# anands-repo/hello

Hardware: AMD Instinct MI355X
Metric: candidate sites/sec (whole node) (higher is better)
Workload: dtype f32

## Files before the change

### hello_amd/csrc/engine.hip

```cpp
#include <hip/hip_runtime.h>

#include <cstdarg>
#include <cstdio>
#include <cstring>
#include <new>
#include <stdexcept>
#include <string>
#include <vector>

#include "../../include/hello_mi355x.h"
#include "kernels.h"

namespace {

thread_local std::string g_last_error;

int fail(int code, const char* fmt, ...) {
    char buf[512];
    va_list ap;
    va_start(ap, fmt);
    vsnprintf(buf, sizeof(buf), fmt, ap);
    va_end(ap);
    g_last_error = buf;
    return code;
}

// ... 100 lines not shown
    DevBuf d_feat_in, d_feat_out;
    DevBuf d_support;
    DevBuf d_evidence;
    hipStream_t own_stream = nullptr;
    hipStream_t last_stream = nullptr;
    hipEvent_t ev_staged = nullptr;
    hipEvent_t ev_start = nullptr, ev_stop = nullptr;
    bool staged_pending = false;
    bool timed = false;
    bool profiling = false;
    std::vector<std::vector<hipEvent_t>> prof_events;
    int prof_count = 0;
    int prof_filter = 0;
    int debug_op = -1;
    DevBuf d_debug;
    size_t debug_floats = 0;
    int stamp_mode = 0;
    DevBuf d_stamps;
    int32_t stamp_layout[5] = {0, 0, 0, 0, 0};

    int32_t *roff0 = nullptr, *roff1 = nullptr, *aoff = nullptr, *site_of_allele = nullptr;
    int32_t *allele_of_read0 = nullptr, *allele_of_read1 = nullptr;
    int32_t *group_slot0 = nullptr, *group_slot1 = nullptr, *slot_off0 = nullptr, *slot_off1 = nullptr;
    hello::ReadConvPlan plan0{1, 0, 0}, plan1{1, 0, 0};
    bool wide_trunk[2] = {false, false};
    int64_t* pair_off = nullptr;
};

namespace {

long long rows_of(int domain, int32_t S, int32_t A, int64_t R0, int64_t R1) {
    switch (domain) {
        case HELLO_ROWS_READS0: return R0;
        case HELLO_ROWS_READS1: return R1;
        case HELLO_ROWS_ALLELES: return A;
        case HELLO_ROWS_SITES: return S;
    }
    return -1;
}

const char* op_name(int kind) {
    static const char* const names[] = {"?", "conv1d", "maxpool", "segsum", "mix", "head", "concat", "add", "readconv_fused",
                                        "layernorm", "compressor_fused", "xattn_front"};
    return kind >= 1 && kind <= HELLO_OP_XATTN_FRONT ? names[kind] : names[0];
}

int validate_op_buffers(const hello_model_desc* d, const hello_op& o, int i) {
    auto domain_of = [&](int id) { return id == HELLO_BUF_READS0 ? (int)HELLO_ROWS_READS0 : id == HELLO_BUF_READS1 ? (int)HELLO_ROWS_READS1
// ... 332 lines not shown
            delete e;
            return fail(HELLO_ERR_MODEL, "a weight block runs past the end of the blob");
        }
    }
    e->scratch.resize(desc->n_buffers);
    hipError_t err = hipMalloc((void**)&e->d_weights, nbytes);
    if (err == hipSuccess) err = hipMemcpy(e->d_weights, folded_weights, nbytes, hipMemcpyHostToDevice);
    if (err == hipSuccess) err = hipStreamCreateWithFlags(&e->own_stream, hipStreamNonBlocking);
    if (err == hipSuccess) err = hipEventCreateWithFlags(&e->ev_staged, hipEventDisableTiming);
    if (err == hipSuccess) err = hipEventCreate(&e->ev_start);
    if (err == hipSuccess) err = hipEventCreate(&e->ev_stop);
    if (err != hipSuccess) {
        hello_engine_destroy(e);
        return fail(HELLO_ERR_HIP, "engine setup failed: %s", hipGetErrorString(err));
    }
    const int n_ops = (int)e->ops.size();
    e->n_lanes = lanes.n_lanes;
    e->partial_of.assign(n_ops, -1);
    int n_partial = e->n_lanes > 1 ? 0 : 2;
    for (int i = 0; i < n_ops; ++i)
        if (e->ops[i].kind == HELLO_OP_READCONV_FUSED)
            e->partial_of[i] = e->n_lanes > 1 ? n_partial++ : (e->ops[i].seg == HELLO_SEG_READS1_TO_ALLELES ? 1 : 0);
    e->d_partial.resize(n_partial);
    if (e->n_lanes > 1) {
        auto lane_of = [&](int i) { return lane_of_op(e->ops[i]); };
        e->op_waits = std::move(lanes.op_waits);
        e->lane_tail = std::move(lanes.lane_tail);
        const std::vector<char>& read_elsewhere = lanes.read_elsewhere;
        e->op_done.assign(n_ops, nullptr);
        e->lane_streams.assign(e->n_lanes, nullptr);
        for (int l = 1; l < e->n_lanes && err == hipSuccess; ++l) err = hipStreamCreateWithFlags(&e->lane_streams[l], hipStreamNonBlocking);
        for (int i = 0; i < n_ops && err == hipSuccess; ++i)
            if (read_elsewhere[i] || (lane_of(i) > 0 && e->lane_tail[lane_of(i)] == i)) err = hipEventCreateWithFlags(&e->op_done[i], hipEventDisableTiming);
        if (err == hipSuccess) err = hipEventCreateWithFlags(&e->ev_lanes_go, hipEventDisableTiming);
        if (err != hipSuccess) {
            hello_engine_destroy(e);
            return fail(HELLO_ERR_HIP, "lane setup failed: %s", hipGetErrorString(err));
        }
    }
    *out = e;
    return HELLO_OK;
} catch (...) {
    return hello::exception_status("hello_engine_create");
}

void hello_engine_destroy(hello_engine* e) {
    if (!e) return;
    (void)hipSetDevice(e->device);
    (void)hipDeviceSynchronize();
    for (auto& b : e->scratch) b.release();
    e->d_csr.release();
    e->h_csr.release();
    e->d_logits.release();
    e->d_meta.release();
    e->d_post.release();
    e->d_out_small.release();
    e->h_io.release();
    e->d_rcl0.release();
    e->d_rcl1.release();
    for (auto& b : e->d_partial) b.release();
    for (hipStream_t st : e->lane_streams)
        if (st) (void)hipStreamDestroy(st);
    for (hipEvent_t ev : e->op_done)
        if (ev) (void)hipEventDestroy(ev);
    if (e->ev_lanes_go) (void)hipEventDestroy(e->ev_lanes_go);
    e->d_feat_in.release();
    e->d_feat_out.release();
    e->d_support.release();
    e->d_evidence.release();
    e->d_debug.release();
    e->d_stamps.release();
    if (e->d_weights) (void)hipFree(e->d_weights);
    if (e->own_stream) (void)hipStreamDestroy(e->own_stream);
    if (e->ev_staged) (void)hipEventDestroy(e->ev_staged);
    if (e->ev_start) (void)hipEventDestroy(e->ev_start);
    if (e->ev_stop) (void)hipEventDestroy(e->ev_stop);
    for (auto& ring : e->prof_events)
        for (auto ev : ring)
            if (ev) (void)hipEventDestroy(ev);
    delete e;
}

void* hello_engine_stream(hello_engine* e) { return e ? (void*)e->own_stream : nullptr; }
// ... 88 lines not shown
    if (capacity < n) return fail(HELLO_ERR_ARG, "capacity %lld < %lld words", (long long)capacity, (long long)n);
    HIP_TRY(hipSetDevice(e->device));
    HIP_TRY(hipStreamSynchronize(e->last_stream ? e->last_stream : e->own_stream));
    HIP_TRY(hipMemcpy(out, e->d_stamps.p, (size_t)n * sizeof(uint64_t), hipMemcpyDeviceToHost));
    return HELLO_OK;
} catch (...) {
    return hello::exception_status("hello_engine_debug_read_stamps");
}

int hello_engine_debug_read(hello_engine* e, float* out, int64_t capacity, int64_t* n_floats) try {
    if (!e || !n_floats) return fail(HELLO_ERR_ARG, "NULL argument");
    *n_floats = (int64_t)e->debug_floats;
    if (!out) return HELLO_OK;
    if (e->debug_floats == 0) return fail(HELLO_ERR_ARG, "no forward has run since hello_engine_debug_capture");
    if (capacity < (int64_t)e->debug_floats) return fail(HELLO_ERR_ARG, "capacity %lld < %zu floats", (long long)capacity, e->debug_floats);
    HIP_TRY(hipSetDevice(e->device));
    HIP_TRY(hipStreamSynchronize(e->last_stream ? e->last_stream : e->own_stream));
    HIP_TRY(hipMemcpy(out, e->d_debug.p, e->debug_floats * sizeof(float), hipMemcpyDeviceToHost));
    return HELLO_OK;
} catch (...) {
    return hello::exception_status("hello_engine_debug_read");
}

static int stage_batch_indices(hello_engine* e, const int32_t* rpa0, const int32_t* rpa1,
                               const int32_t* aps, int32_t S, int32_t A, int64_t R0, int64_t R1,
                               bool two_tech, hipStream_t stream) {
    const int win = hello::readconv_supports_window(e->desc.window) ? e->desc.window : 150;
    const int G = hello::readconv_reads_per_group(win);
    if ((e->wide_trunk[0] || e->wide_trunk[1]) && hello::readconv_wide_reads_per_group() != G)
        return fail(HELLO_ERR_ARG, "internal: the wide trunk's group size differs from the read convolver's");
    const hello::ReadConvPlan plan0 = e->wide_trunk[0] ? hello::readconv_wide_plan(R0) : hello::readconv_plan(R0, win);
    const hello::ReadConvPlan plan1 = !two_tech ? hello::ReadConvPlan{1, 0, 0}
                                      : e->wide_trunk[1] ? hello::readconv_wide_plan(R1) : hello::readconv_plan(R1, win);
    const int64_t n_groups0 = plan0.bulk_wgs + plan0.rest_wgs, n_groups1 = plan1.bulk_wgs + plan1.rest_wgs;
    e->plan0 = plan0;
    e->plan1 = plan1;
    size_t bytes = 0;
    auto add = [&](size_t count, size_t elem) { bytes += (count * elem + 15) & ~size_t(15); };
    add(A + 1, 4); add(A + 1, 4); add(S + 1, 4); add(A, 4);
    add(R0, 4); add(R1, 4);
    add(n_groups0 + 1, 4); add(n_groups1 + 1, 4);
    add(A + 1, 4); add(A + 1, 4);
    add(S + 1, 8);
    if (e->staged_pending) {
        HIP_TRY(hipEventSynchronize(e->ev_staged));
        e->staged_pending = false;
    }
    if (e->h_csr.ensure(bytes)) return fail(HELLO_ERR_HIP, "pinned allocation of %zu bytes failed", bytes);
    if (bytes > e->d_csr.cap) {
        HIP_TRY(hipStreamSynchronize(stream));
        if (e->d_csr.ensure(bytes)) return fail(HELLO_ERR_HIP, "device allocation of %zu bytes failed", bytes);
    }
    char* hc = (char*)e->h_csr.p;
    char* hbase = hc;
    int32_t* h_roff0 = carve<int32_t>(hc, A + 1);
    int32_t* h_roff1 = carve<int32_t>(hc, A + 1);
    int32_t* h_aoff = carve<int32_t>(hc, S + 1);
    int32_t* h_soa = carve<int32_t>(hc, A);
    int32_t* h_aor0 = carve<int32_t>(hc, R0);
    int32_t* h_aor1 = carve<int32_t>(hc, R1);
    int32_t* h_gs0 = carve<int32_t>(hc, n_groups0 + 1);
    int32_t* h_gs1 = carve<int32_t>(hc, n_groups1 + 1);
    int32_t* h_so0 = carve<int32_t>(hc, A + 1);
    int32_t* h_so1 = carve<int32_t>(hc, A + 1);
    int64_t* h_poff = carve<int64_t>(hc, S + 1);

    auto build_reads = [&](const int32_t* rpa, int64_t R, int32_t* roff, int32_t* aor, int32_t* gslot,
                           int32_t* soff, const hello::ReadConvPlan& plan, const char* which) -> int {
        int64_t acc = 0;
        for (int32_t a = 0; a < A; ++a) {
            if (rpa[a] <= 0)
                return fail(HELLO_ERR_SHAPE, "%s[%d] = %d: every allele needs >= 1 read (dummy zero read)",
                            which, a, rpa[a]);
            roff[a] = (int32_t)acc;
            for (int32_t r = 0; r < rpa[a]; ++r) {
                if (acc + r < R) aor[acc + r] = a;
            }
            acc += rpa[a];
            if (acc > R) return fail(HELLO_ERR_SHAPE, "sum(%s) exceeds n_reads = %lld", which, (long long)R);
        }
        roff[A] = (int32_t)acc;
        if (acc != R)
            return fail(HELLO_ERR_SHAPE, "sum(%s) = %lld != n_reads = %lld", which, (long long)acc, (long long)R);
        const int64_t n_wgs = plan.bulk_wgs + plan.rest_wgs;
        const int64_t bulk_reads = plan.rest_wgs ? plan.bulk_wgs * plan.groups_per_wg * G : R;
        for (int32_t a = 0; a <= A; ++a) soff[a] = 0;
        int64_t slot = 0;
        for (int64_t w = 0; w < n_wgs; ++w) {
            int64_t r_lo, r_hi;
            if (w < plan.bulk_wgs) {
                r_lo = w * plan.groups_per_wg * G;
                r_hi = r_lo + (int64_t)plan.groups_per_wg * G;
                if (r_hi > bulk_reads) r_hi = bulk_reads;
            } else {
                r_lo = bulk_reads + (w - plan.bulk_wgs) * G;
                r_hi = r_lo + G < R ? r_lo + G : R;
            }
            if (r_lo >= r_hi) return fail(HELLO_ERR_ARG, "internal: empty workgroup in the read-convolver plan");
            gslot[w] = (int32_t)slot;
            const int32_t first = aor[r_lo], last = aor[r_hi - 1];
            for (int32_t a = first; a <= last; ++a) soff[a + 1] += 1;
            slot += (last - first + 1);
        }
        gslot[n_wgs] = (int32_t)slot;
        int64_t s = 0;
        for (int32_t a = 0; a < A; ++a) {
            const int32_t count = soff[a + 1];
            soff[a] = (int32_t)s;
            s += count;
        }
        soff[A] = (int32_t)s;
        if (s != slot) return fail(HELLO_ERR_ARG, "internal: slot accounting mismatch");
        return 0;
    };
    if (int rc = build_reads(rpa0, R0, h_roff0, h_aor0, h_gs0, h_so0, plan0, "reads_per_allele0")) return rc;
    if (two_tech) {
        if (int rc = build_reads(rpa1, R1, h_roff1, h_aor1, h_gs1, h_so1, plan1, "reads_per_allele1")) return rc;
    } else {
        h_gs1[0] = 0;
    }
    int64_t acc = 0, pacc = 0;
    for (int32_t s = 0; s < S; ++s) {
        if (aps[s] <= 0) return fail(HELLO_ERR_SHAPE, "alleles_per_site[%d] = %d", s, aps[s]);
        h_aoff[s] = (int32_t)acc;
        h_poff[s] = pacc;
        for (int32_t k = 0; k < aps[s] && acc + k < A; ++k) h_soa[acc + k] = s;
        acc += aps[s];
        pacc += (int64_t)aps[s] * (aps[s] + 1) / 2;
        if (acc > A) return fail(HELLO_ERR_SHAPE, "sum(alleles_per_site) exceeds n_alleles = %d", A);
    }
    h_aoff[S] = (int32_t)acc;
    h_poff[S] = pacc;
    if (acc != A) return fail(HELLO_ERR_SHAPE, "sum(alleles_per_site) = %lld != n_alleles = %d", (long long)acc, A);

    HIP_TRY(hipMemcpyAsync(e->d_csr.p, hbase, bytes, hipMemcpyHostToDevice, stream));
    HIP_TRY(hipEventRecord(e->ev_staged, stream));
    e->staged_pending = true;
    char* dbase = (char*)e->d_csr.p;
    auto dev = [&](void* hp) { return dbase + ((char*)hp - hbase); };
    e->roff0 = (int32_t*)dev(h_roff0);
    e->roff1 = (int32_t*)dev(h_roff1);
    e->aoff = (int32_t*)dev(h_aoff);
    e->site_of_allele = (int32_t*)dev(h_soa);
    e->allele_of_read0 = (int32_t*)dev(h_aor0);
    e->allele_of_read1 = (int32_t*)dev(h_aor1);
    e->group_slot0 = (int32_t*)dev(h_gs0);
    e->group_slot1 = (int32_t*)dev(h_gs1);
    e->slot_off0 = (int32_t*)dev(h_so0);
    e->slot_off1 = (int32_t*)dev(h_so1);
    e->pair_off = (int64_t*)dev(h_poff);
    return 0;
}

int hello_engine_forward(hello_engine* e, const uint8_t* reads0, const int32_t* rpa0,
                         const uint8_t* reads1, const int32_t* rpa1, const int32_t* aps,
                         const uint8_t* ref_onehot, int32_t S, int32_t A, int64_t R0, int64_t R1,
                         float* logits, float* meta, float* posteriors, int32_t flags, void* hip_stream) try {
    if (!e) return fail(HELLO_ERR_ARG, "engine is NULL");
    const hello_model_desc& d = e->desc;
    const bool two_tech = d.channels1 > 0;
    if (S <= 0 || A <= 0 || R0 <= 0) return fail(HELLO_ERR_ARG, "empty batch (S=%d A=%d R0=%lld)", S, A, (long long)R0);
    if (A < S) return fail(HELLO_ERR_SHAPE, "n_alleles %d < n_sites %d", A, S);
    if (!reads0 || !rpa0 || !aps || !logits) return fail(HELLO_ERR_ARG, "NULL input/output pointer");
    if (two_tech && (!reads1 || !rpa1 || R1 <= 0)) return fail(HELLO_ERR_ARG, "model needs a second read set");
    if (!two_tech) R1 = 0;
    if (d.uses_ref && !ref_onehot) return fail(HELLO_ERR_ARG, "model needs ref_onehot");
    if (d.has_meta && !meta) return fail(HELLO_ERR_ARG, "model produces meta weights: meta output is NULL");
    if (R0 > 0x7fffffffLL || R1 > 0x7fffffffLL) return fail(HELLO_ERR_ARG, "more than 2^31 reads in one batch");
    HIP_TRY(hipSetDevice(e->device));
    hipStream_t stream = hip_stream ? (hipStream_t)hip_stream : e->own_stream;
// ... 241 lines not shown
                const bool t1 = o.seg == HELLO_SEG_READS1_TO_ALLELES;
                hello::ReadConvArgs a{};
                if (o.flags & HELLO_FLAG_SRC_U8) {
                    a.reads = (const uint8_t*)ptr(o.src0);
                    a.channels = o.cin;
                } else {
                    a.pooled = (const float*)ptr(o.src0);
                }
                if (!ptr(o.src0)) return fail(HELLO_ERR_ARG, "op %d reads an input the caller did not supply", op_index);
                a.w = e->d_weights + o.w_off;
                a.partial = (float*)e->d_partial[e->partial_of[op_index]].p;
                a.allele_of_read = t1 ? e->allele_of_read1 : e->allele_of_read0;
                a.slot_of_group = t1 ? e->group_slot1 : e->group_slot0;
                a.n_reads = t1 ? R1 : R0;
                a.window = d.window;
                a.softplus = (o.flags & HELLO_FLAG_SOFTPLUS) ? 1 : 0;
                a.extra_blocks = o.k;
                a.winograd = (o.flags & HELLO_FLAG_WINOGRAD) ? 1 : 0;
                a.bf16x3 = (o.flags & HELLO_FLAG_BF16X3) ? ((o.flags & HELLO_FLAG_BF16X3_32) ? 2 : 1) : 0;
                const bool wide = o.cout == 128;
                if ((size_t)o.w_off + (wide ? hello::readconv_wide_weight_floats() : hello::readconv_weight_floats(o.k, a.winograd, d.window)) +
                        (a.bf16x3 ? hello::readconv_bf16x3_extra_floats(o.k) : 0) > e->n_weight_floats)
                    return fail(HELLO_ERR_MODEL, "op %d: fused read-convolver weight block truncated", op_index);
                {
                    const hello::ReadConvPlan& plan = t1 ? e->plan1 : e->plan0;
                    const int G = hello::readconv_reads_per_group(d.window);
                    const long long total = a.n_reads;
                    const long long bulk_reads = plan.rest_wgs ? plan.bulk_wgs * plan.groups_per_wg * G : total;
                    a.groups_per_wg = plan.groups_per_wg;
                    a.n_reads = bulk_reads;
                    int32_t stamp_lay[5] = {0, 0, 0, 0, 0};
                    const int stamp_waves = hello::readconv_stamp_waves();
                    if ((e->stamp_mode & 1) && !t1 && total > 0) {
                        if (wide || !a.reads) return fail(HELLO_ERR_ARG, "stamps: the canonical fused read convolver from the bytes only");
                        const long long wgs = plan.rest_wgs ? plan.bulk_wgs + plan.rest_wgs : (long long)((total + (long long)G * plan.groups_per_wg - 1) / ((long long)G * plan.groups_per_wg));
                        const int slots = hello::readconv_stamp_slots();
                        const size_t bytes = (size_t)wgs * stamp_waves * plan.groups_per_wg * slots * sizeof(uint64_t);
                        if (bytes > e->d_stamps.cap) {
                            HIP_TRY(hipStreamSynchronize(stream));
                            if (e->d_stamps.ensure(bytes)) return fail(HELLO_ERR_HIP, "device allocation of %zu bytes failed", bytes);
                        }
                        HIP_TRY(hipMemsetAsync(e->d_stamps.p, 0, bytes, stream));
                        a.stamps = (unsigned long long*)e->d_stamps.p;
                        a.stamp_groups = plan.groups_per_wg;
                        a.stamp_mode = e->stamp_mode;
                        const int32_t lay[5] = {(int32_t)wgs, stamp_waves, plan.groups_per_wg, slots, (int32_t)(plan.rest_wgs ? plan.bulk_wgs : wgs)};
                        for (int i = 0; i < 5; ++i) stamp_lay[i] = lay[i];
                        e->stamp_layout[0] = 0;
                    }
                    HIP_TRY(wide ? hello::launch_readconv_wide(a, stream) : hello::launch_readconv_fused(a, stream));
                    if (plan.rest_wgs) {
                        hello::ReadConvArgs b = a;
                        if (b.stamps) b.stamps += (size_t)plan.bulk_wgs * stamp_waves * plan.groups_per_wg * hello::readconv_stamp_slots();
                        if (b.reads) b.reads += bulk_reads * d.window * o.cin;
                        else b.pooled += bulk_reads * (long long)o.lin * o.cin;
                        b.allele_of_read += bulk_reads;
                        b.slot_of_group += plan.bulk_wgs;
                        b.groups_per_wg = 1;
                        b.n_reads = total - bulk_reads;
                        HIP_TRY(wide ? hello::launch_readconv_wide(b, stream) : hello::launch_readconv_fused(b, stream));
                    }
                    if (a.stamps)
                        for (int i = 0; i < 5; ++i) e->stamp_layout[i] = stamp_lay[i];
                }
                HIP_TRY(hello::launch_readconv_finalize((const float*)e->d_partial[e->partial_of[op_index]].p, t1 ? e->slot_off1 : e->slot_off0,
                                                        (float*)ptr(o.dst), A, o.lout, o.cout, stream));
                break;
            }
        }
        if (op_index == e->debug_op) {
            const size_t per_row = o.kind == HELLO_OP_CONCAT ? (size_t)o.lout * (o.cin + o.c1)
                                   : (o.kind == HELLO_OP_CONV1D || o.kind == HELLO_OP_READCONV_FUSED || o.kind == HELLO_OP_COMPRESSOR_FUSED || o.kind == HELLO_OP_XATTN_FRONT) ? (size_t)o.lout * o.cout
                                   : (o.kind == HELLO_OP_MAXPOOL ? (size_t)o.lout * o.cin : (size_t)o.lin * o.cin);
            const size_t n = (size_t)rows * per_row;
            if (n * sizeof(float) > e->d_debug.cap) {
                HIP_TRY(hipStreamSynchronize(stream));
                if (e->d_debug.ensure(n * sizeof(float))) return fail(HELLO_ERR_HIP, "device allocation of %zu bytes failed", n * sizeof(float));
            }
            HIP_TRY(hipMemcpyAsync(e->d_debug.p, ptr(o.dst), n * sizeof(float), hipMemcpyDeviceToDevice, stream));
            e->debug_floats = n;
        }
        if (laned && e->op_done[op_index]) HIP_TRY(hipEventRecord(e->op_done[op_index], stream));
        ++op_index;
    }
// ... 318 lines not shown
```

### hello_amd/csrc/kernels.h

```cpp
#pragma once
#include <hip/hip_runtime.h>
#include <stdint.h>

namespace hello {

int device_cus();

struct ConvArgs {
    const void* src;
    const float* src2;
    int split;
    float* dst;
    const float* res;
    const float* w;
    const float* bias;
    long long m_total;
    int lin, lout, cin, cout, k, stride, pad;
    int cin_stride;
    int groups;
    int kpad;
    int cout_pad;
    int relu;
    int src_u8;
    unsigned wino_rows;
    int wino;
// ... 18 lines not shown

hipError_t launch_concat(const float* src0, const float* src1, float* dst, long long rows_x_len, int c0,
                         int c1, hipStream_t stream);

hipError_t launch_add(const float* src0, const float* src1, float* dst, long long n, hipStream_t stream);

hipError_t launch_layernorm(const float* src, const float* res, float* dst, const float* gamma, const float* beta,
                            long long positions, int c, float eps, int act, hipStream_t stream);

hipError_t launch_rcl_to_rlc(const uint8_t* src, uint8_t* dst, long long rows, int len, int c,
                             hipStream_t stream);

hipError_t launch_posteriors(const float* logits, const float* meta, const int32_t* allele_off,
                             const int64_t* pair_off, int n_sites, long long n_alleles, int n_experts,
                             long long n_pairs_total, float* out, hipStream_t stream);

struct ReadConvArgs {
    const uint8_t* reads;
    const float* pooled;
    int channels;
    const float* w;
    float* partial;
    const int32_t* allele_of_read;
    const int32_t* slot_of_group;
    int groups_per_wg;
    long long n_reads;
    int extra_blocks;
    int winograd;
    int window;
    int softplus;
    int bf16x3;
    unsigned long long* stamps;
    int stamp_groups;
    int stamp_mode;
};
int readconv_stamp_slots();
int readconv_stamp_waves();
bool readconv_supports_window(int window);
int readconv_reads_per_group(int window);
int readconv_frame_rows(int window);
int readconv_groups_per_workgroup(long long n_reads, int window);
struct ReadConvPlan {
    int groups_per_wg;
    long long bulk_wgs;
    long long rest_wgs;
};
ReadConvPlan readconv_plan(long long n_reads, int window);
ReadConvPlan readconv_wide_plan(long long n_reads);
int readconv_weight_floats(int extra_blocks, bool winograd, int window);
int readconv_bf16x3_extra_floats(int extra_blocks);
bool readconv_supports_extra_blocks(int extra_blocks);
hipError_t launch_readconv_fused(const ReadConvArgs& a, hipStream_t stream);
hipError_t launch_readconv_finalize(const float* partial, const int32_t* slot_off, float* frames, int n_alleles,
                                    int frame_rows, int channels, hipStream_t stream);
int readconv_wide_weight_floats();
int readconv_wide_reads_per_group();
hipError_t launch_readconv_wide(const ReadConvArgs& a, hipStream_t stream);

struct CompressorArgs {
    const float* frames;
    float* dst;
    const float* w;
    long long n_items;
    int blocks;
    int items_per_wg;
};
int small_launch_items_per_wg(long long n_items, int most);
int compressor_weight_floats(int blocks);
bool compressor_supports_blocks(int blocks);
hipError_t launch_compressor_fused(const CompressorArgs& a, hipStream_t stream);
// ... 67 lines not shown
```

### hello_amd/csrc/readconv_fused.hip

```cpp
#include <cstdlib>
#include <type_traits>

#include "kernels.h"

namespace hello {

typedef float f32x4 __attribute__((ext_vector_type(4)));

namespace rc {

constexpr int S1_STEPS = 6;
template <bool WINO, bool F33 = false>
struct Offs {
    static constexpr int KT = WINO ? 4 : 3;
    static constexpr int W3232 = 2 * KT * 2 * 256, W3264 = 4 * 3 * 2 * 256, W3264S = 4 * 1 * 2 * 256;
    static constexpr int W6464 = 4 * KT * 4 * 256;
    static constexpr int W6464D = F33 ? 4 * 5 * 4 * 256 : W6464;
    static constexpr int W3232D = F33 ? 2 * 5 * 2 * 256 : W3232;
    static constexpr int OFF_B = 0;
    static constexpr int OFF_C1 = OFF_B + 6 * (W3232D + 32);
    static constexpr int OFF_SC = OFF_C1 + W3264 + 64;
    static constexpr int OFF_C2 = OFF_SC + W3264S + 64;
    static constexpr int OFF_D = OFF_C2 + W6464D + 64;
    static constexpr int W_TRUNK = OFF_D + 6 * (W6464D + 64);
// ... 44 lines not shown
    static constexpr int NSREG = cmax((T2 * 4 + NW_ - 1) / NW_, 2 * ((RS2 * G_ / 2 + 15) / 16));
    static constexpr int LDS_BYTES = cmax(2 * BUF_FLOATS * 4 + 64 + U8_BYTES,
                                          BUF_FLOATS * 4 + (T2 * 16 + 2) * 256 + 64);
};
}

using Geometry = rc::Cfg<4, 4, 150>;
using Geometry250 = rc::Cfg<2, 4, 250>;
using GeometrySoftplus = rc::Cfg<4, 4, 150, rc::ACT_SOFTPLUS>;
static_assert(Geometry::F33 && GeometrySoftplus::F33 && !Geometry250::F33, "weight packing rule of readconv_pack.py");
static_assert(Geometry::F33_32 && GeometrySoftplus::F33_32, "weight packing rule of readconv_pack.py");
int readconv_bf16x3_extra_floats(int extra_blocks) { return (1 + 2 * (3 + extra_blocks)) * 12288 + 6 * 3072; }
int readconv_weight_floats(int extra_blocks, bool winograd, int window) {
    if (!winograd) return rc::Offs<false>::off_d(3 + extra_blocks);
    return window == 150 ? rc::Offs<true, true>::off_d(3 + extra_blocks) : rc::Offs<true>::off_d(3 + extra_blocks);
}
bool readconv_supports_extra_blocks(int extra_blocks) { return extra_blocks == 0 || extra_blocks == 2; }

bool readconv_supports_window(int window) { return window == 150 || window == 250; }
int readconv_reads_per_group(int window) { return window == 250 ? Geometry250::G : Geometry::G; }
int readconv_stamp_slots() { return rc::STAMP_SLOTS; }
int readconv_stamp_waves() { return Geometry::NW; }
int readconv_frame_rows(int window) { return window == 250 ? Geometry250::L2 : Geometry::L2; }
int readconv_groups_per_workgroup(long long n_reads, int window) {
    const long long slots = 2LL * device_cus();
    const int G = readconv_reads_per_group(window);
    const long long groups = (n_reads + G - 1) / G;
    int best = 1;
    double best_cost = 1e300;
    for (int n = 1; n <= 8; ++n) {
        const long long wgs = (groups + n - 1) / n;
        const double cost = (double)((wgs + slots - 1) / slots) * n * (n > 1 ? 0.988 : 1.0);
        if (cost <= best_cost) {
            best_cost = cost;
            best = n;
        }
    }
    return best;
}

ReadConvPlan readconv_plan(long long n_reads, int window) {
    const long long slots = 2LL * device_cus();
    const int G = readconv_reads_per_group(window);
    const long long groups = (n_reads + G - 1) / G;
    ReadConvPlan best{1, groups, 0};
    double best_cost = 1e300;
    for (int n = 1; n <= 8; ++n) {
        const long long rounds = (groups / n) / slots;
        if (rounds == 0) continue;
        const long long bulk = rounds * slots, rest = groups - bulk * n;
        const double cost = (double)rounds * n * (n > 1 ? 0.988 : 1.0) + (double)((rest + slots - 1) / slots);
        if (cost <= best_cost) {
            best_cost = cost;
            best = ReadConvPlan{n, bulk, rest};
        }
    }
    if (best_cost == 1e300) {
        const int n = readconv_groups_per_workgroup(n_reads, window);
        best = ReadConvPlan{n, (groups + n - 1) / n, 0};
    }
    return best;
}

template <int C>
__device__ __forceinline__ int swz(int row) {
    return (C == 64 || C == 128) ? 2 * (row & 7) : (C == 32 ? 2 * ((row >> 1) & 3) : 2 * ((row >> 2) & 1));
}

enum { SW_OLD = 0, SW_W = 1, SW_3 = 2, SW_SPLIT = 3, SW_GLOBAL = 4 };

typedef short bf16x8 __attribute__((ext_vector_type(8)));
typedef short bf16x4 __attribute__((ext_vector_type(4)));
__device__ __forceinline__ int split_off(int row, int g, int part) { return row * 256 + 16 * ((g + 8 * part) ^ (2 * (row & 7))); }
__device__ __forceinline__ unsigned short to_bf16(float x) {
    const __bf16 h = (__bf16)x;
    return __builtin_bit_cast(unsigned short, h);
}
__device__ __forceinline__ int split_off32(int row, int g, int part) { return row * 128 + 16 * ((g + 4 * part) ^ (2 * ((row >> 1) & 3))); }
__device__ __forceinline__ void split4(f32x4 v, bf16x4& h, bf16x4& l) {
#pragma unroll
    for (int e = 0; e < 4; ++e) {
        const unsigned short hi = to_bf16(v[e]);
        h[e] = (short)hi;
        l[e] = (short)to_bf16(v[e] - __uint_as_float((unsigned)hi << 16));
    }
// ... 1000 lines not shown
    {
        const int j = tid0 & 15;
        const int pg1 = wave0 / 2;
        if (WINO) {
#pragma unroll
            for (int k = 0; k < (T1 / 2 + 1) / 2; ++k) {
                pad1 |= ((((pg1 + 2 * k) * 16 + j) % (RS1 / 2)) == RS1 / 2 - 1 ? 1u : 0u) << k;
                pad1f |= ((((1 - pg1 + 2 * k) * 16 + j) % (RS1 / 2)) == RS1 / 2 - 1 ? 1u : 0u) << k;
            }
        } else {
#pragma unroll
            for (int k = 0; k < T1 / 2; ++k) pad1 |= ((((pg1 + 2 * k) * 16 + j) % RS1) >= L1 ? 1u : 0u) << k;
        }
    }

    float* const X = STEM ? bufB : bufA;
    float* const H = STEM ? bufA : bufB;
    f32x4 sreg[CF::NSREG];
    f32x4 wA[NVA], wB[NVB], w2[2];
    f32x4 w3[2][5];
    f32x4 (&w6)[6] = reinterpret_cast<f32x4 (&)[6]>(wA);
    f32x4 (&w12)[12] = reinterpret_cast<f32x4 (&)[12]>(wB);

    const long long wg_read0 = (long long)blockIdx.x * G * a.groups_per_wg;
    const int slot0 = a.slot_of_group[blockIdx.x];
    const int first_allele = a.allele_of_read[wg_read0];
    int cur = first_allele;
    constexpr int NF = (L2 * 16 + THREADS - 1) / THREADS;
    f32x4 carry[NF];
#pragma unroll
    for (int i = 0; i < NF; ++i) carry[i] = f32x4{0.f, 0.f, 0.f, 0.f};
    auto flush = [&]() {
#pragma unroll
        for (int i = 0; i < NF; ++i) {
            const int f = tid0 + THREADS * i;
            if (f < L2 * 16)
                *(f32x4*)(a.partial + ((long long)(slot0 + cur - first_allele) * L2 + (f >> 4)) * 64 + 4 * (f & 15)) = carry[i];
            carry[i] = f32x4{0.f, 0.f, 0.f, 0.f};
        }
    };

    for (int grp = 0; grp < a.groups_per_wg; ++grp) {
    int opaque_zero;
    asm volatile("s_mov_b32 %0, 0" : "=s"(opaque_zero));
    const int tid = tid0 + opaque_zero;
    const int wave = __builtin_amdgcn_readfirstlane(wave0 + opaque_zero);
    const int lane = tid & 63;
    const int cb2 = wave % 2, cb4 = wave;
    const long long read0 = wg_read0 + (long long)grp * G;
    if (read0 >= a.n_reads) break;
    unsigned long long* const stamp_base = STAMP ? a.stamps + (((long long)blockIdx.x * CF::NW + wave) * a.stamp_groups + grp) * STAMP_SLOTS : nullptr;
    auto stamp = [&](int slot) {
        if constexpr (STAMP) {
            const unsigned long long t = __builtin_amdgcn_s_memtime();
            if (grp < a.stamp_groups && lane == 0) stamp_base[slot] = t;
        }
    };
    auto barrier = [&](int id) {
        stamp(1 + 2 * id);
        __syncthreads();
        stamp(2 + 2 * id);
    };
    if constexpr (STAMP) {
        stamp(0);
        const unsigned long long rt = __builtin_amdgcn_s_memrealtime();
        const unsigned hw = __builtin_amdgcn_s_getreg((31 << 11) | 4), xcc = __builtin_amdgcn_s_getreg((31 << 11) | 20);
        if (grp < a.stamp_groups && lane == 0) {
            stamp_base[41] = (unsigned long long)hw | ((unsigned long long)xcc << 32);
            stamp_base[42] = rt;
        }
    }
    const int n_here = (int)((a.n_reads - read0) < G ? (a.n_reads - read0) : G);
    if constexpr (F33) {
        static_assert(!F33 || CF::F33_32, "the F(3,3) kernel runs its 32-channel blocks in F(3,3) form too");
// ... 211 lines not shown
            else
                wino_layer<CF, 64, MODE_RESID_INPLACE, false>(H, X, wB, nullptr, W + off_b + W6464, pad2w, dump, wave, lane);
        } else {
            conv_layer<CF, 64, 64, 3, 1, 1, RS2, RS2, L2, T2, MODE_PLAIN, true, GEOM_TRUNK, 16, RS2 * CF::G, true>(
                X, H, w12, slice(off_b, cb4, 12), W + off_a + W6464, sreg, pad2, dump, wave, lane);
            barrier(13 + 2 * blk);
            if (blk < NB64 - 1)
                conv_layer<CF, 64, 64, 3, 1, 1, RS2, RS2, L2, T2, MODE_RESID_INPLACE, true, GEOM_TRUNK, 16, RS2 * CF::G, true>(
                    H, X, w12, slice(O::off_d(blk + 1), cb4, 12), W + off_b + W6464, sreg, pad2, dump, wave, lane);
            else
                conv_layer<CF, 64, 64, 3, 1, 1, RS2, RS2, L2, T2, MODE_RESID_INPLACE, false, GEOM_TRUNK, 16, RS2 * CF::G, true>(
                    H, X, w12, nullptr, W + off_b + W6464, sreg, pad2, dump, wave, lane);
        }
        barrier(14 + 2 * blk);
    }

    static_assert(G <= 4, "the allele select below");
    int allele_of[G];
#pragma unroll
    for (int rd = 0; rd < G; ++rd) {
        const long long r = read0 + rd < a.n_reads ? read0 + rd : a.n_reads - 1;
        allele_of[rd] = __builtin_amdgcn_readfirstlane(a.allele_of_read[r]);
    }
#pragma nounroll
    for (int rd = 0; rd < n_here; ++rd) {
        const int al = rd == 0 ? allele_of[0] : rd == 1 ? allele_of[1 % G] : rd == 2 ? allele_of[2 % G] : allele_of[3 % G];
        if (al != cur) {
            flush();
            cur = al;
        }
#pragma unroll
        for (int i = 0; i < NF; ++i) {
            const int f = tid + THREADS * i;
            if (f < L2 * 16) {
                const f32x4 v = *(const f32x4*)(X + img_off<64, F33 ? SW_3 : SWX>(1 + rd * RS2 + (f >> 4), f & 15));
#pragma unroll
                for (int e = 0; e < 4; ++e) carry[i][e] += v[e];
            }
        }
    }
    barrier(19);
    if constexpr (STAMP) {
        const unsigned long long rt = __builtin_amdgcn_s_memrealtime();
        if (grp < a.stamp_groups && lane == 0) stamp_base[43] = rt;
    }
    }
    flush();
    if constexpr (STAMP) {
        static_assert(!STAMP || (NB64 == 3 && STEM && WINO && !BF16), "stamps: the default fp32 Winograd schedule (20 barriers per group)");
        const unsigned long long t = __builtin_amdgcn_s_memtime();
        if ((tid0 & 63) == 0) a.stamps[(((long long)blockIdx.x * CF::NW + wave0) * a.stamp_groups) * STAMP_SLOTS + 44] = t;
    }
}

template <class CF, int NB64, bool WINO, bool STEM_ONLY = false, bool BF16 = false, bool BF16_32 = false>
static hipError_t launch_cfg(const ReadConvArgs& a, hipStream_t stream) {
    static bool configured_on[64] = {};
    int dev = 0;
    if (hipGetDevice(&dev) != hipSuccess || dev < 0 || dev >= 64) return hipErrorInvalidDevice;
    bool& configured = configured_on[dev];
    if (!configured) {
        hipError_t e = hipSuccess;
        if constexpr (!STEM_ONLY)
            e = hipFuncSetAttribute((const void*)readconv_kernel<CF, false, NB64, WINO, BF16, BF16_32>,
                                    hipFuncAttributeMaxDynamicSharedMemorySize, CF::LDS_BYTES);
        if (e == hipSuccess)
            e = hipFuncSetAttribute((const void*)readconv_kernel<CF, true, NB64, WINO, BF16, BF16_32>,
                                    hipFuncAttributeMaxDynamicSharedMemorySize, CF::LDS_BYTES);
        if (e != hipSuccess) return e;
        configured = true;
    }
    if (a.groups_per_wg < 1) return hipErrorInvalidValue;
    const long long per_wg = (long long)CF::G * a.groups_per_wg;
    const unsigned groups = (unsigned)((a.n_reads + per_wg - 1) / per_wg);
    if (a.stamps) {
        if constexpr (std::is_same<CF, Geometry>::value && NB64 == 3 && WINO && !BF16 && !STEM_ONLY) {
            if (!a.reads || (a.channels != 6 && a.channels != 7) || a.stamp_groups < 1) return hipErrorInvalidValue;
            static bool stamped_on[64] = {};
            if (!stamped_on[dev]) {
                const hipError_t e = hipFuncSetAttribute((const void*)readconv_kernel<CF, true, NB64, WINO, false, false, true>,
                                                         hipFuncAttributeMaxDynamicSharedMemorySize, 100 * 1024);
                if (e != hipSuccess) return e;
                stamped_on[dev] = true;
            }
            const int lds = (a.stamp_mode & 2) ? 100 * 1024 : CF::LDS_BYTES;
            hipLaunchKernelGGL((readconv_kernel<CF, true, NB64, WINO, false, false, true>), dim3(groups), dim3(CF::THREADS), lds, stream, a);
            return hipGetLastError();
        } else {
            return hipErrorInvalidValue;
        }
    }
    if (a.reads) {
        if (a.channels != 6 && a.channels != 7) return hipErrorInvalidValue;
        hipLaunchKernelGGL((readconv_kernel<CF, true, NB64, WINO, BF16, BF16_32>), dim3(groups), dim3(CF::THREADS), CF::LDS_BYTES, stream, a);
    } else if constexpr (!STEM_ONLY) {
        hipLaunchKernelGGL((readconv_kernel<CF, false, NB64, WINO, BF16, BF16_32>), dim3(groups), dim3(CF::THREADS), CF::LDS_BYTES, stream, a);
    } else {
// ... 705 lines not shown
```

Before: 487,000.

## Replace static read-convolver workgroup plan with persistent chunked scheduling via atomic counter

The fused read convolver previously ran a bulk launch plus a remainder launch with a fixed number of groups per workgroup. It now builds a host-side list of chunks whose sizes taper toward the end, launches one persistent grid sized to the resident slots, and has each workgroup pull its next chunk from an atomic counter. This removes the second launch and aims to balance the tail across CUs. The cost is an extra memset and atomic per chunk, a loop around the kernel body that may raise register pressure, and an optional env cap on slots.

```diff
diff --git a/hello_amd/csrc/engine.hip b/hello_amd/csrc/engine.hip
--- a/hello_amd/csrc/engine.hip
+++ b/hello_amd/csrc/engine.hip
@@ -2,6 +2,7 @@
 
 #include <cstdarg>
 #include <cstdio>
+#include <cstdlib>
 #include <cstring>
 #include <new>
 #include <stdexcept>
@@ -148,8 +149,11 @@
     int32_t *roff0 = nullptr, *roff1 = nullptr, *aoff = nullptr, *site_of_allele = nullptr;
     int32_t *allele_of_read0 = nullptr, *allele_of_read1 = nullptr;
     int32_t *group_slot0 = nullptr, *group_slot1 = nullptr, *slot_off0 = nullptr, *slot_off1 = nullptr;
-    hello::ReadConvPlan plan0{1, 0, 0}, plan1{1, 0, 0};
     bool wide_trunk[2] = {false, false};
+    hello::ReadConvChunkPlan chunk_plan[2];
+    hello::ReadConvChunk* chunks[2] = {nullptr, nullptr};
+    int readconv_slots_cap = 0;
+    DevBuf d_counters;
     int64_t* pair_off = nullptr;
 };
 
@@ -528,6 +532,19 @@
         if (e->ops[i].kind == HELLO_OP_READCONV_FUSED)
             e->partial_of[i] = e->n_lanes > 1 ? n_partial++ : (e->ops[i].seg == HELLO_SEG_READS1_TO_ALLELES ? 1 : 0);
     e->d_partial.resize(n_partial);
+    if (e->d_counters.ensure((size_t)(n_ops > 0 ? n_ops : 1) * 64)) {
+        hello_engine_destroy(e);
+        return fail(HELLO_ERR_HIP, "device allocation of the chunk counters failed");
+    }
+    if (const char* cap = getenv("HELLO_READCONV_SLOTS")) {
+        char* end = nullptr;
+        const long v = strtol(cap, &end, 10);
+        if (end == cap || *end || v < 1 || v > (1 << 20)) {
+            hello_engine_destroy(e);
+            return fail(HELLO_ERR_ARG, "HELLO_READCONV_SLOTS = '%s': a count of resident workgroups >= 1", cap);
+        }
+        e->readconv_slots_cap = (int)v;
+    }
     if (e->n_lanes > 1) {
         auto lane_of = [&](int i) { return lane_of_op(e->ops[i]); };
         e->op_waits = std::move(lanes.op_waits);
@@ -565,6 +582,7 @@
     e->d_rcl0.release();
     e->d_rcl1.release();
     for (auto& b : e->d_partial) b.release();
+    e->d_counters.release();
     for (hipStream_t st : e->lane_streams)
         if (st) (void)hipStreamDestroy(st);
     for (hipEvent_t ev : e->op_done)
@@ -699,6 +717,11 @@
     return hello::exception_status("hello_engine_debug_read");
 }
 
+static long long readconv_slots(const hello_engine* e, int per_cu) {
+    const long long device = hello::readconv_resident_slots(per_cu);
+    return e->readconv_slots_cap > 0 && e->readconv_slots_cap < device ? e->readconv_slots_cap : device;
+}
+
 static int stage_batch_indices(hello_engine* e, const int32_t* rpa0, const int32_t* rpa1,
                                const int32_t* aps, int32_t S, int32_t A, int64_t R0, int64_t R1,
                                bool two_tech, hipStream_t stream) {
@@ -706,17 +729,19 @@
     const int G = hello::readconv_reads_per_group(win);
     if ((e->wide_trunk[0] || e->wide_trunk[1]) && hello::readconv_wide_reads_per_group() != G)
         return fail(HELLO_ERR_ARG, "internal: the wide trunk's group size differs from the read convolver's");
-    const hello::ReadConvPlan plan0 = e->wide_trunk[0] ? hello::readconv_wide_plan(R0) : hello::readconv_plan(R0, win);
-    const hello::ReadConvPlan plan1 = !two_tech ? hello::ReadConvPlan{1, 0, 0}
-                                      : e->wide_trunk[1] ? hello::readconv_wide_plan(R1) : hello::readconv_plan(R1, win);
-    const int64_t n_groups0 = plan0.bulk_wgs + plan0.rest_wgs, n_groups1 = plan1.bulk_wgs + plan1.rest_wgs;
-    e->plan0 = plan0;
-    e->plan1 = plan1;
+    const long long slots = readconv_slots(e, 2);
+    const int64_t groups0 = (R0 + G - 1) / G, groups1 = two_tech ? (R1 + G - 1) / G : 0;
+    const bool chunked0 = !e->wide_trunk[0], chunked1 = two_tech && !e->wide_trunk[1];
+    e->chunk_plan[0] = chunked0 ? hello::readconv_chunk_plan(groups0, slots) : hello::ReadConvChunkPlan{};
+    e->chunk_plan[1] = chunked1 ? hello::readconv_chunk_plan(groups1, slots) : hello::ReadConvChunkPlan{};
+    const int64_t n_groups0 = chunked0 ? 0 : groups0, n_groups1 = chunked1 ? 0 : groups1;
+    const int64_t n_chunks0 = e->chunk_plan[0].chunks, n_chunks1 = e->chunk_plan[1].chunks;
     size_t bytes = 0;
     auto add = [&](size_t count, size_t elem) { bytes += (count * elem + 15) & ~size_t(15); };
     add(A + 1, 4); add(A + 1, 4); add(S + 1, 4); add(A, 4);
     add(R0, 4); add(R1, 4);
     add(n_groups0 + 1, 4); add(n_groups1 + 1, 4);
+    add(n_chunks0, sizeof(hello::ReadConvChunk)); add(n_chunks1, sizeof(hello::ReadConvChunk));
     add(A + 1, 4); add(A + 1, 4);
     add(S + 1, 8);
     if (e->staged_pending) {
@@ -738,12 +763,14 @@
     int32_t* h_aor1 = carve<int32_t>(hc, R1);
     int32_t* h_gs0 = carve<int32_t>(hc, n_groups0 + 1);
     int32_t* h_gs1 = carve<int32_t>(hc, n_groups1 + 1);
+    hello::ReadConvChunk* h_ch0 = carve<hello::ReadConvChunk>(hc, n_chunks0);
+    hello::ReadConvChunk* h_ch1 = carve<hello::ReadConvChunk>(hc, n_chunks1);
     int32_t* h_so0 = carve<int32_t>(hc, A + 1);
     int32_t* h_so1 = carve<int32_t>(hc, A + 1);
     int64_t* h_poff = carve<int64_t>(hc, S + 1);
 
-    auto build_reads = [&](const int32_t* rpa, int64_t R, int32_t* roff, int32_t* aor, int32_t* gslot,
-                           int32_t* soff, const hello::ReadConvPlan& plan, const char* which) -> int {
+    auto build_reads = [&](const int32_t* rpa, int64_t R, int32_t* roff, int32_t* aor, int32_t* gslot, hello::ReadConvChunk* chunks,
+                           int64_t n_expected, int32_t* soff, const char* which) -> int {
         int64_t acc = 0;
         for (int32_t a = 0; a < A; ++a) {
             if (rpa[a] <= 0)
@@ -759,27 +786,31 @@
         roff[A] = (int32_t)acc;
         if (acc != R)
             return fail(HELLO_ERR_SHAPE, "sum(%s) = %lld != n_reads = %lld", which, (long long)acc, (long long)R);
-        const int64_t n_wgs = plan.bulk_wgs + plan.rest_wgs;
-        const int64_t bulk_reads = plan.rest_wgs ? plan.bulk_wgs * plan.groups_per_wg * G : R;
         for (int32_t a = 0; a <= A; ++a) soff[a] = 0;
-        int64_t slot = 0;
-        for (int64_t w = 0; w < n_wgs; ++w) {
-            int64_t r_lo, r_hi;
-            if (w < plan.bulk_wgs) {
-                r_lo = w * plan.groups_per_wg * G;
-                r_hi = r_lo + (int64_t)plan.groups_per_wg * G;
-                if (r_hi > bulk_reads) r_hi = bulk_reads;
-            } else {
-                r_lo = bulk_reads + (w - plan.bulk_wgs) * G;
-                r_hi = r_lo + G < R ? r_lo + G : R;
+        int64_t slot = 0, n_units = 0;
+        bool empty = false;
+        auto unit = [&](long long first_group, int n_groups) {
+            const int64_t r_lo = first_group * G, r_hi = r_lo + (int64_t)n_groups * G < R ? r_lo + (int64_t)n_groups * G : R;
+            if (r_lo >= r_hi) {
+                empty = true;
+                return;
             }
-            if (r_lo >= r_hi) return fail(HELLO_ERR_ARG, "internal: empty workgroup in the read-convolver plan");
-            gslot[w] = (int32_t)slot;
+            if (chunks) chunks[n_units] = hello::ReadConvChunk{(int32_t)first_group, (int32_t)n_groups, (int32_t)slot};
+            else gslot[n_units] = (int32_t)slot;
             const int32_t first = aor[r_lo], last = aor[r_hi - 1];
             for (int32_t a = first; a <= last; ++a) soff[a + 1] += 1;
             slot += (last - first + 1);
-        }
-        gslot[n_wgs] = (int32_t)slot;
+            n_units += 1;
+        };
+        const int64_t groups = (R + G - 1) / G;
+        if (chunks) {
+            hello::readconv_for_each_chunk(groups, slots, unit);
+            if (n_units != n_expected) return fail(HELLO_ERR_ARG, "internal: the read convolver's chunk list changed length");
+        } else {
+            for (int64_t w = 0; w < groups; ++w) unit(w, 1);
+            gslot[n_units] = (int32_t)slot;
+        }
+        if (empty) return fail(HELLO_ERR_ARG, "internal: empty chunk in the read-convolver plan");
         int64_t s = 0;
         for (int32_t a = 0; a < A; ++a) {
             const int32_t count = soff[a + 1];
@@ -790,9 +821,9 @@
         if (s != slot) return fail(HELLO_ERR_ARG, "internal: slot accounting mismatch");
         return 0;
     };
-    if (int rc = build_reads(rpa0, R0, h_roff0, h_aor0, h_gs0, h_so0, plan0, "reads_per_allele0")) return rc;
+    if (int rc = build_reads(rpa0, R0, h_roff0, h_aor0, h_gs0, chunked0 ? h_ch0 : nullptr, n_chunks0, h_so0, "reads_per_allele0")) return rc;
     if (two_tech) {
-        if (int rc = build_reads(rpa1, R1, h_roff1, h_aor1, h_gs1, h_so1, plan1, "reads_per_allele1")) return rc;
+        if (int rc = build_reads(rpa1, R1, h_roff1, h_aor1, h_gs1, chunked1 ? h_ch1 : nullptr, n_chunks1, h_so1, "reads_per_allele1")) return rc;
     } else {
         h_gs1[0] = 0;
     }
@@ -823,6 +854,8 @@
     e->allele_of_read1 = (int32_t*)dev(h_aor1);
     e->group_slot0 = (int32_t*)dev(h_gs0);
     e->group_slot1 = (int32_t*)dev(h_gs1);
+    e->chunks[0] = (hello::ReadConvChunk*)dev(h_ch0);
+    e->chunks[1] = (hello::ReadConvChunk*)dev(h_ch1);
     e->slot_off0 = (int32_t*)dev(h_so0);
     e->slot_off1 = (int32_t*)dev(h_so1);
     e->pair_off = (int64_t*)dev(h_poff);
@@ -1110,44 +1143,35 @@
                 if ((size_t)o.w_off + (wide ? hello::readconv_wide_weight_floats() : hello::readconv_weight_floats(o.k, a.winograd, d.window)) +
                         (a.bf16x3 ? hello::readconv_bf16x3_extra_floats(o.k) : 0) > e->n_weight_floats)
                     return fail(HELLO_ERR_MODEL, "op %d: fused read-convolver weight block truncated", op_index);
-                {
-                    const hello::ReadConvPlan& plan = t1 ? e->plan1 : e->plan0;
-                    const int G = hello::readconv_reads_per_group(d.window);
-                    const long long total = a.n_reads;
-                    const long long bulk_reads = plan.rest_wgs ? plan.bulk_wgs * plan.groups_per_wg * G : total;
-                    a.groups_per_wg = plan.groups_per_wg;
-                    a.n_reads = bulk_reads;
+                if (wide) {
+                    if ((e->stamp_mode & 1) && !t1) return fail(HELLO_ERR_ARG, "stamps: the canonical fused read convolver from the bytes only");
+                    a.groups_per_wg = 1;
+                    HIP_TRY(hello::launch_readconv_wide(a, stream));
+                } else {
+                    const hello::ReadConvChunkPlan& plan = e->chunk_plan[t1 ? 1 : 0];
+                    a.chunks = e->chunks[t1 ? 1 : 0];
+                    a.n_chunks = (int)plan.chunks;
+                    a.counter = (unsigned*)((char*)e->d_counters.p + (size_t)op_index * 64);
+                    const bool stamped = (e->stamp_mode & 1) && !t1 && a.n_reads > 0;
+                    a.resident_slots = (int)readconv_slots(e, stamped && (e->stamp_mode & 2) ? 1 : 2);
                     int32_t stamp_lay[5] = {0, 0, 0, 0, 0};
-                    const int stamp_waves = hello::readconv_stamp_waves();
-                    if ((e->stamp_mode & 1) && !t1 && total > 0) {
-                        if (wide || !a.reads) return fail(HELLO_ERR_ARG, "stamps: the canonical fused read convolver from the bytes only");
-                        const long long wgs = plan.rest_wgs ? plan.bulk_wgs + plan.rest_wgs : (long long)((total + (long long)G * plan.groups_per_wg - 1) / ((long long)G * plan.groups_per_wg));
-                        const int slots = hello::readconv_stamp_slots();
-                        const size_t bytes = (size_t)wgs * stamp_waves * plan.groups_per_wg * slots * sizeof(uint64_t);
+                    if (stamped) {
+                        if (!a.reads) return fail(HELLO_ERR_ARG, "stamps: the canonical fused read convolver from the bytes only");
+                        const int stamp_waves = hello::readconv_stamp_waves(), slots = hello::readconv_stamp_slots();
+                        const size_t bytes = (size_t)plan.chunks * stamp_waves * plan.head * slots * sizeof(uint64_t);
                         if (bytes > e->d_stamps.cap) {
                             HIP_TRY(hipStreamSynchronize(stream));
                             if (e->d_stamps.ensure(bytes)) return fail(HELLO_ERR_HIP, "device allocation of %zu bytes failed", bytes);
                         }
                         HIP_TRY(hipMemsetAsync(e->d_stamps.p, 0, bytes, stream));
                         a.stamps = (unsigned long long*)e->d_stamps.p;
-                        a.stamp_groups = plan.groups_per_wg;
+                        a.stamp_groups = plan.head;
                         a.stamp_mode = e->stamp_mode;
-                        const int32_t lay[5] = {(int32_t)wgs, stamp_waves, plan.groups_per_wg, slots, (int32_t)(plan.rest_wgs ? plan.bulk_wgs : wgs)};
+                        const int32_t lay[5] = {(int32_t)plan.chunks, stamp_waves, plan.head, slots, (int32_t)plan.bulk};
                         for (int i = 0; i < 5; ++i) stamp_lay[i] = lay[i];
                         e->stamp_layout[0] = 0;
                     }
-                    HIP_TRY(wide ? hello::launch_readconv_wide(a, stream) : hello::launch_readconv_fused(a, stream));
-                    if (plan.rest_wgs) {
-                        hello::ReadConvArgs b = a;
-                        if (b.stamps) b.stamps += (size_t)plan.bulk_wgs * stamp_waves * plan.groups_per_wg * hello::readconv_stamp_slots();
-                        if (b.reads) b.reads += bulk_reads * d.window * o.cin;
-                        else b.pooled += bulk_reads * (long long)o.lin * o.cin;
-                        b.allele_of_read += bulk_reads;
-                        b.slot_of_group += plan.bulk_wgs;
-                        b.groups_per_wg = 1;
-                        b.n_reads = total - bulk_reads;
-                        HIP_TRY(wide ? hello::launch_readconv_wide(b, stream) : hello::launch_readconv_fused(b, stream));
-                    }
+                    HIP_TRY(hello::launch_readconv_fused(a, stream));
                     if (a.stamps)
                         for (int i = 0; i < 5; ++i) e->stamp_layout[i] = stamp_lay[i];
                 }
diff --git a/hello_amd/csrc/kernels.h b/hello_amd/csrc/kernels.h
--- a/hello_amd/csrc/kernels.h
+++ b/hello_amd/csrc/kernels.h
@@ -1,6 +1,8 @@
 #pragma once
 #include <hip/hip_runtime.h>
 #include <stdint.h>
+
+#include "readconv_chunks.h"
 
 namespace hello {
 
@@ -65,6 +67,10 @@
     const float* w;
     float* partial;
     const int32_t* allele_of_read;
+    const ReadConvChunk* chunks;
+    int n_chunks;
+    unsigned* counter;
+    int resident_slots;
     const int32_t* slot_of_group;
     int groups_per_wg;
     long long n_reads;
@@ -82,13 +88,12 @@
 bool readconv_supports_window(int window);
 int readconv_reads_per_group(int window);
 int readconv_frame_rows(int window);
-int readconv_groups_per_workgroup(long long n_reads, int window);
 struct ReadConvPlan {
     int groups_per_wg;
     long long bulk_wgs;
     long long rest_wgs;
 };
-ReadConvPlan readconv_plan(long long n_reads, int window);
+long long readconv_resident_slots(int per_cu = 2);
 ReadConvPlan readconv_wide_plan(long long n_reads);
 int readconv_weight_floats(int extra_blocks, bool winograd, int window);
 int readconv_bf16x3_extra_floats(int extra_blocks);
diff --git a/hello_amd/csrc/readconv_chunks.h b/hello_amd/csrc/readconv_chunks.h
--- /dev/null
+++ b/hello_amd/csrc/readconv_chunks.h
@@ -0,0 +1,66 @@
+#pragma once
+
+#include <cstdint>
+
+namespace hello {
+
+constexpr int READCONV_MAX_CHUNK = 8;
+constexpr int READCONV_TAPER_ROUNDS = 2;
+
+struct ReadConvChunk {
+    int32_t first_group;
+    int32_t groups;
+    int32_t first_slot;
+};
+
+struct ReadConvChunkPlan {
+    int head = 1;
+    long long chunks = 0;
+    long long bulk = 0;
+    bool counter = false;
+};
+
+inline int readconv_head_groups(long long groups, long long slots) {
+    int best = 1;
+    double best_cost = 1e300;
+    for (int n = 1; n <= READCONV_MAX_CHUNK; ++n) {
+        const long long rounds = (groups / n) / slots;
+        if (rounds == 0) continue;
+        const long long rest = groups - rounds * slots * n;
+        const double cost = (double)rounds * n * (n > 1 ? 0.988 : 1.0) + (double)((rest + slots - 1) / slots);
+        if (cost <= best_cost) {
+            best_cost = cost;
+            best = n;
+        }
+    }
+    return best;
+}
+
+template <class F>
+inline ReadConvChunkPlan readconv_for_each_chunk(long long groups, long long slots, F&& f) {
+    ReadConvChunkPlan p;
+    if (groups <= 0) return p;
+    if (slots < 1) slots = 1;
+    p.head = readconv_head_groups(groups, slots);
+    const long long div = (long long)READCONV_TAPER_ROUNDS * slots;
+    int largest = 0;
+    for (long long g = 0; g < groups;) {
+        const long long left = groups - g;
+        long long n = (left + div - 1) / div;
+        if (n > p.head) n = p.head;
+        f(g, (int)n);
+        if ((int)n > largest) largest = (int)n;
+        p.chunks += 1;
+        p.bulk += n > 1;
+        g += n;
+    }
+    p.head = largest;
+    p.counter = p.chunks > slots;
+    return p;
+}
+
+inline ReadConvChunkPlan readconv_chunk_plan(long long groups, long long slots) {
+    return readconv_for_each_chunk(groups, slots, [](long long, int) {});
+}
+
+}
diff --git a/hello_amd/csrc/readconv_fused.hip b/hello_amd/csrc/readconv_fused.hip
--- a/hello_amd/csrc/readconv_fused.hip
+++ b/hello_amd/csrc/readconv_fused.hip
@@ -90,45 +90,7 @@
 int readconv_stamp_slots() { return rc::STAMP_SLOTS; }
 int readconv_stamp_waves() { return Geometry::NW; }
 int readconv_frame_rows(int window) { return window == 250 ? Geometry250::L2 : Geometry::L2; }
-int readconv_groups_per_workgroup(long long n_reads, int window) {
-    const long long slots = 2LL * device_cus();
-    const int G = readconv_reads_per_group(window);
-    const long long groups = (n_reads + G - 1) / G;
-    int best = 1;
-    double best_cost = 1e300;
-    for (int n = 1; n <= 8; ++n) {
-        const long long wgs = (groups + n - 1) / n;
-        const double cost = (double)((wgs + slots - 1) / slots) * n * (n > 1 ? 0.988 : 1.0);
-        if (cost <= best_cost) {
-            best_cost = cost;
-            best = n;
-        }
-    }
-    return best;
-}
-
-ReadConvPlan readconv_plan(long long n_reads, int window) {
-    const long long slots = 2LL * device_cus();
-    const int G = readconv_reads_per_group(window);
-    const long long groups = (n_reads + G - 1) / G;
-    ReadConvPlan best{1, groups, 0};
-    double best_cost = 1e300;
-    for (int n = 1; n <= 8; ++n) {
-        const long long rounds = (groups / n) / slots;
-        if (rounds == 0) continue;
-        const long long bulk = rounds * slots, rest = groups - bulk * n;
-        const double cost = (double)rounds * n * (n > 1 ? 0.988 : 1.0) + (double)((rest + slots - 1) / slots);
-        if (cost <= best_cost) {
-            best_cost = cost;
-            best = ReadConvPlan{n, bulk, rest};
-        }
-    }
-    if (best_cost == 1e300) {
-        const int n = readconv_groups_per_workgroup(n_reads, window);
-        best = ReadConvPlan{n, (groups + n - 1) / n, 0};
-    }
-    return best;
-}
+long long readconv_resident_slots(int per_cu) { return (long long)per_cu * device_cus(); }
 
 template <int C>
 __device__ __forceinline__ int swz(int row) {
@@ -1175,14 +1137,16 @@
     f32x4 (&w6)[6] = reinterpret_cast<f32x4 (&)[6]>(wA);
     f32x4 (&w12)[12] = reinterpret_cast<f32x4 (&)[12]>(wB);
 
-    const long long wg_read0 = (long long)blockIdx.x * G * a.groups_per_wg;
-    const int slot0 = a.slot_of_group[blockIdx.x];
+    __shared__ int next_chunk;
+    constexpr int NF = (L2 * 16 + THREADS - 1) / THREADS;
+    f32x4 carry[NF];
+#pragma unroll
+    for (int i = 0; i < NF; ++i) carry[i] = f32x4{0.f, 0.f, 0.f, 0.f};
+    for (int chunk = blockIdx.x; chunk < a.n_chunks;) {
+    const int chunk_groups = a.chunks[chunk].groups, slot0 = a.chunks[chunk].first_slot;
+    const long long wg_read0 = (long long)a.chunks[chunk].first_group * G;
     const int first_allele = a.allele_of_read[wg_read0];
     int cur = first_allele;
-    constexpr int NF = (L2 * 16 + THREADS - 1) / THREADS;
-    f32x4 carry[NF];
-#pragma unroll
-    for (int i = 0; i < NF; ++i) carry[i] = f32x4{0.f, 0.f, 0.f, 0.f};
     auto flush = [&]() {
 #pragma unroll
         for (int i = 0; i < NF; ++i) {
@@ -1193,7 +1157,8 @@
         }
     };
 
-    for (int grp = 0; grp < a.groups_per_wg; ++grp) {
+    int next = a.n_chunks;
+    for (int grp = 0; grp < chunk_groups; ++grp) {
     int opaque_zero;
     asm volatile("s_mov_b32 %0, 0" : "=s"(opaque_zero));
     const int tid = tid0 + opaque_zero;
@@ -1202,7 +1167,7 @@
     const int cb2 = wave % 2, cb4 = wave;
     const long long read0 = wg_read0 + (long long)grp * G;
     if (read0 >= a.n_reads) break;
-    unsigned long long* const stamp_base = STAMP ? a.stamps + (((long long)blockIdx.x * CF::NW + wave) * a.stamp_groups + grp) * STAMP_SLOTS : nullptr;
+    unsigned long long* const stamp_base = STAMP ? a.stamps + (((long long)chunk * CF::NW + wave) * a.stamp_groups + grp) * STAMP_SLOTS : nullptr;
     auto stamp = [&](int slot) {
         if constexpr (STAMP) {
             const unsigned long long t = __builtin_amdgcn_s_memtime();
@@ -1460,6 +1425,9 @@
         const long long r = read0 + rd < a.n_reads ? read0 + rd : a.n_reads - 1;
         allele_of[rd] = __builtin_amdgcn_readfirstlane(a.allele_of_read[r]);
     }
+    const bool pull = a.counter != nullptr && grp == chunk_groups - 1;
+    int pulled = 0;
+    if (pull && tid == 0) pulled = (int)(gridDim.x + atomicAdd(a.counter, 1u));
 #pragma nounroll
     for (int rd = 0; rd < n_here; ++rd) {
         const int al = rd == 0 ? allele_of[0] : rd == 1 ? allele_of[1 % G] : rd == 2 ? allele_of[2 % G] : allele_of[3 % G];
@@ -1477,7 +1445,9 @@
             }
         }
     }
+    if (pull && tid == 0) next_chunk = pulled;
     barrier(19);
+    if (pull) next = __builtin_amdgcn_readfirstlane(next_chunk);
     if constexpr (STAMP) {
         const unsigned long long rt = __builtin_amdgcn_s_memrealtime();
         if (grp < a.stamp_groups && lane == 0) stamp_base[43] = rt;
@@ -1487,12 +1457,14 @@
     if constexpr (STAMP) {
         static_assert(!STAMP || (NB64 == 3 && STEM && WINO && !BF16), "stamps: the default fp32 Winograd schedule (20 barriers per group)");
         const unsigned long long t = __builtin_amdgcn_s_memtime();
-        if ((tid0 & 63) == 0) a.stamps[(((long long)blockIdx.x * CF::NW + wave0) * a.stamp_groups) * STAMP_SLOTS + 44] = t;
+        if ((tid0 & 63) == 0) a.stamps[(((long long)chunk * CF::NW + wave0) * a.stamp_groups) * STAMP_SLOTS + 44] = t;
+    }
+    chunk = next;
     }
 }
 
 template <class CF, int NB64, bool WINO, bool STEM_ONLY = false, bool BF16 = false, bool BF16_32 = false>
-static hipError_t launch_cfg(const ReadConvArgs& a, hipStream_t stream) {
+static hipError_t launch_cfg(const ReadConvArgs& a_in, hipStream_t stream) {
     static bool configured_on[64] = {};
     int dev = 0;
     if (hipGetDevice(&dev) != hipSuccess || dev < 0 || dev >= 64) return hipErrorInvalidDevice;
@@ -1508,9 +1480,17 @@
         if (e != hipSuccess) return e;
         configured = true;
     }
-    if (a.groups_per_wg < 1) return hipErrorInvalidValue;
-    const long long per_wg = (long long)CF::G * a.groups_per_wg;
-    const unsigned groups = (unsigned)((a.n_reads + per_wg - 1) / per_wg);
+    if (!a_in.chunks || a_in.n_chunks < 1 || a_in.resident_slots < 1) return hipErrorInvalidValue;
+    ReadConvArgs a = a_in;
+    unsigned groups = (unsigned)a.n_chunks;
+    if (a.n_chunks > a.resident_slots) {
+        if (!a.counter) return hipErrorInvalidValue;
+        const hipError_t e = hipMemsetAsync(a.counter, 0, sizeof(unsigned), stream);
+        if (e != hipSuccess) return e;
+        groups = (unsigned)a.resident_slots;
+    } else {
+        a.counter = nullptr;
+    }
     if (a.stamps) {
         if constexpr (std::is_same<CF, Geometry>::value && NB64 == 3 && WINO && !BF16 && !STEM_ONLY) {
             if (!a.reads || (a.channels != 6 && a.channels != 7) || a.stamp_groups < 1) return hipErrorInvalidValue;
```

Result: no change. 491,100, median of 6 (+0.8%).
